# Ssellu/vslam-pose-estimation-framework

Hardware: AMD Instinct MI355X
Metric: stereo frames/sec on KITTI-00 at 1/2/4/8 MI355X; ATE vs reference (higher is better)
Workload: dtype u8

## Files before the change

vslam_pose_estimation_framework_amd/csrc/host_ctx.h:

```cpp
#pragma once

static thread_local std::string g_create_error;

#ifndef VS_SPLIT4_MAX_STREAMS
#define VS_SPLIT4_MAX_STREAMS 96
#endif
struct vslam_ctx {
  DevCfg cfg;
  DevBuf buf;
  int device = 0;
  int B = 0;
  hipStream_t stream = nullptr;
  hipStream_t stream_img = nullptr;
  bool own_stream = false;
  hipEvent_t ev_img[2] = {nullptr, nullptr}, ev_frm[2] = {nullptr, nullptr};
  bool frm_pending[2] = {false, false};
  int q0_frm = 0, q0_img = 0;
  struct ImgSet { uint16_t* box; uint8_t* score8; unsigned long long* mask; int16_t* kp_xy; uint8_t* kp_score; uint8_t* desc;
                  int32_t* n_kp; int32_t* rowcell; uint8_t* used; uint8_t* sdist; ImgInfo* iinfo; } sets[2];
  int parity = 0, last_set = 0;
  std::string err;
  std::vector<void*> allocs;
  DevCfg* d_cfg = nullptr;
  DevBuf* d_bufs = nullptr;
// ... 304 lines not shown
static void destroy_streams(vslam_ctx* c) {
  for (int q = 0; q < 2; ++q) {
    if (c->ev_img[q]) (void)hipEventDestroy(c->ev_img[q]);
    if (c->ev_frm[q]) (void)hipEventDestroy(c->ev_frm[q]);
    c->ev_img[q] = c->ev_frm[q] = nullptr;
  }
  if (c->own_stream) {
    if (c->stream_img && c->stream_img != c->stream) (void)hipStreamDestroy(c->stream_img);
    if (c->stream) (void)hipStreamDestroy(c->stream);
  }
  c->stream = c->stream_img = nullptr;
}
__global__ void k_xcc_probe(int* out) {
  unsigned v;
  asm volatile("s_getreg_b32 %0, hwreg(HW_REG_XCC_ID)" : "=s"(v));
  if (threadIdx.x == 0) *out = (int)(v & 7u);
}
static int calibrate_queues(vslam_ctx* c) {
  int* d = nullptr;
  if (hipMalloc(&d, 2 * sizeof(int)) != hipSuccess) return VSLAM_OK;
  int h[2] = {0, 0};
  hipStream_t q[2] = {c->stream, c->stream_img};
  bool ok = true;
  for (int k = 0; k < 2 && ok; ++k) { hipLaunchKernelGGL(k_xcc_probe, dim3(1), dim3(64), 0, q[k], d + k); ok = hipStreamSynchronize(q[k]) == hipSuccess; }
  if (ok && hipMemcpy(h, d, sizeof h, hipMemcpyDeviceToHost) == hipSuccess) { c->q0_frm = h[0]; c->q0_img = h[1]; }
  (void)hipFree(d);
  return VSLAM_OK;
}

static int create_internal(const vslam_config* cfg, int device, int n_streams, vslam_ctx** out) {
  if (!cfg || !out || n_streams < 1) return fail(nullptr, VSLAM_ERR_INVALID, "vslam_create: null argument or n_streams < 1");
  if (n_streams > VS_MAX_STREAMS) return fail(nullptr, VSLAM_ERR_INVALID, "vslam_create: more than 4096 streams in one context");
  if (cfg->rows < 1 || cfg->cols < 1 || cfg->cols > 32767 || cfg->rows > 32767) return fail(nullptr, VSLAM_ERR_INVALID, "vslam_create: invalid image dimensions");
  if (cfg->det_rows < 1 || cfg->det_cols < 1 || cfg->det_rows * cfg->det_cols > VSLAM_MAX_REGIONS) return fail(nullptr, VSLAM_ERR_INVALID, "vslam_create: invalid detector grid");
  if (!(-cfg->baseline_h[0] / cfg->K[0] > 0)) return fail(nullptr, VSLAM_ERR_INVALID, "vslam_create: invalid baseline (m), verify intrinsic camera parameters");
  if (cfg->maximum_epipolar_search_offset_pixels < 0 || cfg->maximum_epipolar_search_offset_pixels > VSLAM_MAX_EPI) return fail(nullptr, VSLAM_ERR_INVALID, "vslam_create: epipolar offset out of range");
  if (cfg->descriptor_type != VSLAM_DESCRIPTOR_BRIEF && cfg->descriptor_type != VSLAM_DESCRIPTOR_ORB) return fail(nullptr, VSLAM_ERR_INVALID, "vslam_create: unknown descriptor_type");
  if (cfg->max_keypoints < 64 || cfg->max_keypoints > 65535 || cfg->max_points < 64 || cfg->max_history_frames < 2 || cfg->bin_size_pixels < 1) return fail(nullptr, VSLAM_ERR_INVALID, "vslam_create: invalid capacities");
  int ndev = 0;
  if (hipGetDeviceCount(&ndev) != hipSuccess || ndev < 1) return fail(nullptr, VSLAM_ERR_NO_DEVICE, "vslam_create: no HIP device available (the HIP path has no CPU fallback)");
  if (device < 0 || device >= ndev) return fail(nullptr, VSLAM_ERR_NO_DEVICE, "vslam_create: device ordinal out of range");
  if (hipSetDevice(device) != hipSuccess) return fail(nullptr, VSLAM_ERR_NO_DEVICE, "vslam_create: hipSetDevice failed");
  hipFuncAttributes fa;
  if (hipFuncGetAttributes(&fa, reinterpret_cast<const void*>(k_frame)) != hipSuccess)
    return fail(nullptr, VSLAM_ERR_NO_DEVICE, "vslam_create: no gfx950 kernel image for this device");
  vslam_ctx* c = new vslam_ctx;
  c->device = device;
  c->B = n_streams;
  derive_cfg(*cfg, n_streams, &c->cfg);
  {
    bool ok = hipStreamCreateWithPriority(&c->stream, hipStreamNonBlocking, 0) == hipSuccess &&
              hipStreamCreateWithPriority(&c->stream_img, hipStreamNonBlocking, 0) == hipSuccess;
    if (ok && getenv("VSLAM_IMG_STREAMS") && atoi(getenv("VSLAM_IMG_STREAMS")) == 0) { (void)hipStreamDestroy(c->stream_img); c->stream_img = c->stream; }
    for (int k = 0; k < 2 && ok; ++k)
      ok = hipEventCreateWithFlags(&c->ev_img[k], hipEventDisableTiming) == hipSuccess &&
           hipEventCreateWithFlags(&c->ev_frm[k], hipEventDisableTiming) == hipSuccess;
    c->own_stream = true;
    if (!ok) { destroy_streams(c); delete c; return fail(nullptr, VSLAM_ERR_HIP, "hipStreamCreate failed"); }
    c->split = n_streams <= VS_SPLIT4_MAX_STREAMS ? 4 : 0;
    if (const char* e = getenv("VSLAM_SPLIT")) { const int v = atoi(e); if (v == 0 || v == 4) c->split = v; }
  }
  const DevCfg& d = c->cfg;
  DevBuf& b = c->buf;
  std::memset(&b, 0, sizeof b);
  std::memset(b.active, 0xff, sizeof b.active);
  const size_t B = n_streams, S2 = B * 2, rows = cfg->rows, N = d.NMAX, P = d.MAXP, Hc = d.HCAP;
// ... 242 lines not shown
```

vslam_pose_estimation_framework_amd/csrc/host_frame.h:

```cpp
#pragma once

static int report_blocks(int what) {
  return what == VS_REPORT_KEYPOINTS ? 32 : what == VS_REPORT_POINTS ? 16 : what == VS_REPORT_KEYPOINTS_XY ? 8 : 4;
}
static int report_launch(vslam_ctx* c, hipStream_t q, const DevBuf& bs, int s, int what, int in_progress) {
  const int seq = ++c->report_seq;
  hipLaunchKernelGGL(k_report, dim3(report_blocks(what)), dim3(256), 0, q, c->cfg, bs, s, what, in_progress, seq, c->rl, c->report_dev, c->report_done);
  return seq;
}
static int launch_image_pipeline(vslam_ctx* c) {
  const DevCfg& d = c->cfg;
  const int set = c->parity;
  const int n = c->B;
  hipStream_t st = c->img_override ? c->img_override : c->stream_img;
  if (!c->img_override && c->img_on_frm_queue) {
    HIP_TRY(c, hipStreamSynchronize(c->stream));
    c->img_on_frm_queue = false;
  }
  if (c->img_override) c->img_on_frm_queue = true;
  const bool coarse = c->img_override != nullptr;
  if (c->frm_pending[set] && st != c->stream) HIP_TRY(c, hipStreamWaitEvent(st, c->ev_frm[set], 0));
  HIP_TRY(c, prestage_enqueue(st, c->pre, c->rect.maps, c->eq, n, 2, c->buf.active));
  const bool masked = c->dmask.pending || c->dmask.stat[0] || c->dmask.stat[1];
  if (masked) { if (const int rc = mask_prepare(c, st)) return rc; } else c->dmask.last = 0;
// ... 142 lines not shown
  p.smooth_mode = c->sm.mode; p.smooth_ksize = c->sm.ksize;
  const ImgPlanes raw_slab = p.remap ? ImgPlanes{{r.raw[set][0], r.raw[set][1]}, r.raw_stride, r.raw_stream_stride} : p.smooth_mode ? unsmoothed_planes(c, set) : up;
  if (p.format != VSLAM_PIXEL_GRAY8) { p.color = cur; p.gray = p.factor > 1 ? ImgPlanes{{d.full[set][0], d.full[set][1]}, d.stride, d.stream_stride} : raw_slab; cur = p.gray; }
  if (p.factor > 1) { p.full = cur; p.reduced = raw_slab; cur = p.reduced; }
  if (p.remap) { p.raw = cur; p.mapped = rectified_planes(c, set); cur = p.mapped; }
  if (p.smooth_mode) { p.unsmoothed = cur; p.smoothed = c->eq.on ? ImgPlanes{{c->sm.out[0], c->sm.out[1]}, c->up_stride, c->up_stream_stride} : up; cur = p.smoothed; }
  if (c->eq.on) { c->eq.src = cur; c->eq.dst = cur.p[0] == up.p[0] ? cur : up; cur = c->eq.dst; }
  buf_set_planes(c->buf, cur);
}
static int set_inputs(vslam_ctx* c, const uint8_t* L, const uint8_t* R, int32_t row_stride, size_t image_stride, bool on_device) {
  const bool colour = c->col.format != VSLAM_PIXEL_GRAY8, full = c->ds.factor > 1, raw = c->rect.on;
  int rows, cols;
  incoming_size(c, &rows, &cols);
  const int wb = colour ? gray_channels(c->col.format) * cols : cols;
  if (!L || !R) return fail(c, VSLAM_ERR_INVALID, "called with empty frame");
  if (row_stride < wb)
    return fail(c, VSLAM_ERR_INVALID, colour ? "row stride smaller than channels * image width" : full ? "row stride smaller than the full image width" : raw ? "row stride smaller than the raw image width" : "row stride smaller than image width");
  ImgPlanes in = {{L, R}, row_stride, image_stride};
  if (!on_device) {
    if (colour && c->mapcol.rgb && c->frm_pending[c->parity]) {
      hipStream_t up[2] = {c->img_override ? c->img_override : c->stream_img, c->stream_img};
      for (int k = 0; k < 2; ++k)
        if (up[k] != c->stream && (k == 0 || up[k] != up[0])) HIP_TRY(c, hipStreamWaitEvent(up[k], c->ev_frm[c->parity], 0));
    }
    const int p = c->parity;
    const int rc = colour ? upload_to(c, L, R, row_stride, image_stride, rows, wb, c->col.slab[p], c->col.stride, c->col.stream_stride, &in)
                   : full ? upload_to(c, L, R, row_stride, image_stride, rows, cols, c->ds.full[p], c->ds.stride, c->ds.stream_stride, &in)
                   : raw  ? upload_to(c, L, R, row_stride, image_stride, rows, cols, c->rect.raw[p], c->rect.raw_stride, c->rect.raw_stream_stride, &in)
                   : c->sm.mode ? upload_to(c, L, R, row_stride, image_stride, rows, cols, c->sm.in[p], c->up_stride, c->up_stream_stride, &in)
                          : upload_to(c, L, R, row_stride, image_stride, rows, cols, c->upload[p], c->up_stride, c->up_stream_stride, &in);
    if (rc != VSLAM_OK) return rc;
  }
  route_frame(c, in);
  return VSLAM_OK;
}

static int process_frame(vslam_ctx* c, const uint8_t* L, const uint8_t* R, int32_t row_stride, size_t image_stride, bool on_device) {
  if (!c) return VSLAM_ERR_INVALID;
  if (c->sticky != VSLAM_OK) return c->sticky;
  if (!on_device) HIP_TRY(c, hipSetDevice(c->device));
  int rc = set_inputs(c, L, R, row_stride, image_stride, on_device);
  if (rc != VSLAM_OK) return rc;
  rc = flush_pending(c);
  if (rc != VSLAM_OK) return rc;
  rc = launch_image_pipeline(c);
  if (rc != VSLAM_OK) return rc;
  return launch_frame(c);
}
VS_API int vslam_process_device(vslam_ctx* c, const uint8_t* L, const uint8_t* R, int32_t row_stride, size_t image_stride) {
  return process_frame(c, L, R, row_stride, image_stride, true);
}
VS_API int vslam_process_host(vslam_ctx* c, const uint8_t* L, const uint8_t* R, int32_t row_stride, size_t image_stride) {
  return process_frame(c, L, R, row_stride, image_stride, false);
}

VS_API int vslam_host_alloc(void** out, size_t bytes) {
  if (!out || !bytes) return VSLAM_ERR_INVALID;
  void* p = nullptr;
  if (hipHostMalloc(&p, bytes, hipHostMallocDefault) != hipSuccess) { (void)hipGetLastError(); return fail(nullptr, VSLAM_ERR_HIP, "vslam_host_alloc: hipHostMalloc failed"); }
  *out = p;
  return VSLAM_OK;
}
VS_API void vslam_host_free(void* p) { if (p) (void)hipHostFree(p); }
```

vslam_pose_estimation_framework_amd/csrc/host_rgbd.h:

```cpp
#pragma once
#include "rgbd_tracker.h"
#include "rgbd_device.h"
struct vslam_rgbd {
  bool on_host = false, host_pending = false;
  int host_rc = 0;
  vs_rgbd::Tracker t;
  vs_rgbd::DeviceTracker d;
  std::string& err() { return on_host ? t.err : d.err; }
};
static thread_local std::string g_rgbd_error;
VS_API const char* vslam_rgbd_last_error(const vslam_rgbd* r) { return r ? (r->on_host ? r->t.err.c_str() : r->d.err.c_str()) : g_rgbd_error.c_str(); }
static int rgbd_create(const vslam_config* cfg, const vslam_depth_params* p, int device, int n_streams, vslam_rgbd** out) {
  if (!cfg || !p || !out) { g_rgbd_error = "vslam_rgbd_create: null argument"; return VSLAM_ERR_INVALID; }
  vslam_rgbd* r = new vslam_rgbd;
  if (const char* e = std::getenv("VSLAM_RGBD_HOST")) r->on_host = std::atoi(e) != 0;
  if (p->detector_type == VSLAM_DETECTOR_ORB) { if (!vs_rgbd::DeviceTracker::orb_grid_supported(*cfg)) r->on_host = true; }
  else if (p->detector_type != VSLAM_DETECTOR_FAST) { g_rgbd_error = "vslam_rgbd_create: unknown detector_type"; delete r; return VSLAM_ERR_INVALID; }
  if (r->on_host && n_streams != 1) { g_rgbd_error = "vslam_rgbd_create_batch: the host-driven loop (VSLAM_RGBD_HOST=1, detector_type ORB on a grid above 2 x 2) tracks one sequence per object"; delete r; return VSLAM_ERR_INVALID; }
  const int rc = r->on_host ? r->t.create(*cfg, *p, device) : r->d.create(*cfg, *p, device, n_streams);
  if (rc != VSLAM_OK) { g_rgbd_error = r->err(); delete r; return rc; }
  *out = r;
  return VSLAM_OK;
}
VS_API int vslam_rgbd_create(const vslam_config* cfg, const vslam_depth_params* p, int device, vslam_rgbd** out) { return rgbd_create(cfg, p, device, 1, out); }
VS_API int vslam_rgbd_create_batch(const vslam_config* cfg, const vslam_depth_params* p, int device, int32_t n_streams, vslam_rgbd** out) {
  return rgbd_create(cfg, p, device, n_streams, out);
}
VS_API void vslam_rgbd_destroy(vslam_rgbd* r) { delete r; }
VS_API int vslam_rgbd_reset(vslam_rgbd* r) {
  if (!r) return VSLAM_ERR_INVALID;
  if (r->on_host) { r->t.reset(); return VSLAM_OK; }
  return r->d.reset();
}
static int rgbd_frame_args_ok(vslam_rgbd* r, const uint8_t* left, int32_t lstride, const uint16_t* depth, int32_t dstride) {
  if (!left || !depth) { r->err() = "called with empty frame"; return VSLAM_ERR_INVALID; }
  const int cols = r->on_host ? r->t.cfg.cols : r->d.in_cols();
  const int wb = r->on_host ? cols : r->d.in_bytes();
  if (lstride < wb || dstride < cols) { r->err() = "row stride smaller than image width"; return VSLAM_ERR_INVALID; }
  return VSLAM_OK;
}
VS_API int vslam_rgbd_process_host(vslam_rgbd* r, const uint8_t* left, int32_t lstride, const uint16_t* depth, int32_t dstride) {
  if (!r) return VSLAM_ERR_INVALID;
  if (int rc = rgbd_frame_args_ok(r, left, lstride, depth, dstride)) return rc;
  return r->on_host ? r->t.process(left, lstride, depth, dstride) : r->d.process(left, lstride, depth, dstride);
}
VS_API int vslam_rgbd_submit_host(vslam_rgbd* r, const uint8_t* left, int32_t lstride, const uint16_t* depth, int32_t dstride) {
  if (!r) return VSLAM_ERR_INVALID;
  if (int rc = rgbd_frame_args_ok(r, left, lstride, depth, dstride)) return rc;
  if (r->on_host) { r->host_rc = r->t.process(left, lstride, depth, dstride); r->host_pending = true; return r->host_rc; }
  return r->d.submit(left, lstride, depth, dstride);
}
VS_API int vslam_rgbd_wait(vslam_rgbd* r) {
  if (!r) return VSLAM_ERR_INVALID;
  if (r->on_host) {
    if (!r->host_pending) { r->t.err = "RGB-D tracker: no frame in flight"; return VSLAM_ERR_STATE; }
    r->host_pending = false;
    return r->host_rc;
  }
  return r->d.wait();
}
VS_API int vslam_rgbd_submit_batch_host(vslam_rgbd* r, const uint8_t* left, int32_t lstride, size_t left_stream_stride, const uint16_t* depth, int32_t dstride,
                                        size_t depth_stream_stride) {
  if (!r) return VSLAM_ERR_INVALID;
  if (r->on_host) { r->t.err = "batch entry points need the device-resident loop"; return VSLAM_ERR_STATE; }
  if (int rc = rgbd_frame_args_ok(r, left, lstride, depth, dstride)) return rc;
  return r->d.submit(left, lstride, depth, dstride, left_stream_stride, depth_stream_stride);
}
VS_API int vslam_rgbd_process_batch_host(vslam_rgbd* r, const uint8_t* left, int32_t lstride, size_t left_stream_stride, const uint16_t* depth, int32_t dstride,
                                         size_t depth_stream_stride) {
  const int rc = vslam_rgbd_submit_batch_host(r, left, lstride, left_stream_stride, depth, dstride, depth_stream_stride);
  return rc != VSLAM_OK ? rc : vslam_rgbd_wait(r);
// ... 248 lines not shown
```

vslam_pose_estimation_framework_amd/csrc/kernels_image.h:

```cpp
#pragma once
#include <hip/hip_runtime.h>
#include "dev_types.h"
#include "../../include/vslam_brief_pattern.h"
#include "../../include/vslam_orb_pattern.h"
#include "brief_footprint.h"

__constant__ int8_t c_brief[256][4] = VSLAM_BRIEF_PATTERN_INIT;
constexpr int8_t k_brief_builtin[256][4] = VSLAM_BRIEF_PATTERN_INIT;
constexpr BriefFootprint k_brief_builtin_fp = brief_footprint(k_brief_builtin);
__constant__ BriefFootprint c_brief_fp = k_brief_builtin_fp;
__constant__ int8_t c_orb[256][4] = VSLAM_ORB_PATTERN_INIT;

__device__ __forceinline__ size_t ix_side(const DevCfg& c, int s, int d) { return (size_t)s * 2 + d; }
__device__ __forceinline__ uint16_t* box_of(const DevCfg& c, const DevBuf& b, int s, int d) {
  return b.box + ix_side(c, s, d) * (size_t)c.c.rows * c.bstride;
}
__device__ __forceinline__ uint8_t* score_of(const DevCfg& c, const DevBuf& b, int s, int d) {
  return b.score8 + ix_side(c, s, d) * (size_t)c.c.rows * c.bstride;
}
__device__ __forceinline__ unsigned long long* mask_of(const DevCfg& c, const DevBuf& b, int s, int d) {
  return b.mask + ix_side(c, s, d) * (size_t)c.c.rows * c.TX;
}
__device__ __forceinline__ int16_t* kpxy_of(const DevCfg& c, const DevBuf& b, int s, int d) {
  return b.kp_xy + ix_side(c, s, d) * (size_t)c.NMAX * 2;
}
__device__ __forceinline__ uint8_t* kpscore_of(const DevCfg& c, const DevBuf& b, int s, int d) {
  return b.kp_score + ix_side(c, s, d) * (size_t)c.NMAX;
}
__device__ __forceinline__ uint8_t* desc_of(const DevCfg& c, const DevBuf& b, int s, int d) {
  return b.desc + ix_side(c, s, d) * (size_t)c.NMAX * 32;
}
__device__ __forceinline__ int32_t* rowcell_of(const DevCfg& c, const DevBuf& b, int s, int d) {
  return b.rowcell + ix_side(c, s, d) * (size_t)c.c.rows * (c.CW + 1);
}
__device__ __forceinline__ uint8_t* used_of(const DevCfg& c, const DevBuf& b, int s, int d) {
  return b.used + ix_side(c, s, d) * (size_t)c.NMAX;
}
__device__ __forceinline__ int32_t* kill_of(const DevCfg& c, const DevBuf& b, int s, int d) {
  return b.kill + ix_side(c, s, d) * (size_t)c.NMAX;
}

__device__ __forceinline__ int block_exclusive_scan(int v, int* sh, int* total) {
  const int lane = threadIdx.x & 63, w = threadIdx.x >> 6, nw = blockDim.x >> 6;
  int inc = v;
#pragma unroll
  for (int o = 1; o < 64; o <<= 1) {
    const int t = __shfl_up(inc, o, 64);
    if (lane >= o) inc += t;
  }
  __syncthreads();
  if (lane == 63) sh[w] = inc;
  __syncthreads();
  if (threadIdx.x == 0) {
    int acc = 0;
    for (int i = 0; i < nw; ++i) { const int t = sh[i]; sh[i] = acc; acc += t; }
    sh[16] = acc;
  }
  __syncthreads();
  *total = sh[16];
  return sh[w] + inc - v;
}

__device__ __forceinline__ void xcd_tile(int* tx, int* ty, int* tz, int mono = 0, int rot = 0) {
  const int gx = gridDim.x, gy = gridDim.y;
  const int tps = mono ? gx * gy : gx * gy * 2;
  const int ns = mono ? gridDim.z : gridDim.z >> 1;
  int lin = blockIdx.x + gx * (blockIdx.y + gy * blockIdx.z);
  const int per = (ns >> 3) * tps;
  if (lin < (per << 3)) { const int x = (lin + rot) & 7, j = lin >> 3, q = j / tps; lin = (x + 8 * q) * tps + (j - q * tps); }
  *tx = lin % gx;
  const int r = lin / gx;
  *ty = r % gy;
// ... 45 lines not shown
__device__ __forceinline__ int lds_fetch_add(int* word, int v) {
  const uint32_t addr = (uint32_t)reinterpret_cast<uintptr_t>((__attribute__((address_space(3))) int*)word);
  int old;
  asm volatile("ds_add_rtn_u32 %0, %1, %2\n\ts_waitcnt lgkmcnt(0)" : "=&v"(old) : "v"(addr), "v"(v) : "memory");
  return old;
}

#define VS_FB_QCAP ((VS_TILE_H + 2) * 66)
#define VS_FB_HS_BYTES ((VS_TILE_H + 8) * VS_TILE_W * 2)
#define VS_FB_DYN_LDS ((VS_FB_QCAP * 2) > VS_FB_HS_BYTES ? (VS_FB_QCAP * 2) : VS_FB_HS_BYTES)
__global__ __launch_bounds__(256, 8) void k_fast_box(const DevCfg c, const DevBuf b) {
  extern __shared__ __align__(16) unsigned char fb_dyn[];
  __shared__ __align__(16) uint8_t tile[VS_TILE_H + 8][80];
  __shared__ __align__(4) uint8_t sc[VS_TILE_H + 2][68];
  __shared__ int32_t s_thr[VSLAM_MAX_REGIONS];
  uint16_t* queue = reinterpret_cast<uint16_t*>(fb_dyn);
  uint16_t (*hs)[VS_TILE_W] = reinterpret_cast<uint16_t (*)[VS_TILE_W]>(fb_dyn);
  __shared__ unsigned long long lmask[VS_TILE_H];
  __shared__ int qn;
  int tx, ty, tz;
  xcd_tile(&tx, &ty, &tz, c.mono, b.xcd_rot);
  const int s = b.s0 + (c.mono ? tz : (tz >> 1)), side = c.mono ? 0 : (tz & 1);
  if (!vs_active(b, s)) return;
  const int x0 = tx * VS_TILE_W, y0 = ty * VS_TILE_H;
  const int rows = c.c.rows, cols = c.c.cols;
  const uint8_t* img = b.img[side] + (size_t)s * b.img_stream_stride;
  const int stride = b.img_row_stride;
  const int tid = threadIdx.x, lane = tid & 63, w = tid >> 6;
  if (tid < c.n_regions) s_thr[tid] = min(max(b.st[s].thr[tid], 0), 255);
  if (tid == 0) qn = 0;
  if (tid < VS_TILE_H) lmask[tid] = 0ull;
  for (int i = tid; i < (VS_TILE_H + 2) * 17; i += 256) reinterpret_cast<uint32_t*>(&sc[0][0])[i] = 0u;
  const bool aligned = ((stride & 3) == 0) && ((reinterpret_cast<uintptr_t>(img) & 3) == 0);
  constexpr int NST = ((VS_TILE_H + 8) * 18 + 255) / 256;
  if (aligned && x0 >= 4 && x0 + 68 <= cols) {
    uint32_t v[NST];
#pragma unroll
    for (int u = 0; u < NST; ++u) {
      const int i = tid + 256 * u;
      const int r = i / 18, q = i - r * 18;
      const int gy = min(max(y0 - 4 + r, 0), rows - 1);
      v[u] = 0;
      if (i < (VS_TILE_H + 8) * 18) v[u] = __builtin_nontemporal_load(reinterpret_cast<const uint32_t*>(img + (size_t)gy * stride + (x0 - 4 + 4 * q)));
    }
#pragma unroll
    for (int u = 0; u < NST; ++u) {
      const int i = tid + 256 * u;
      const int r = i / 18, q = i - r * 18;
      if (i < (VS_TILE_H + 8) * 18) *reinterpret_cast<uint32_t*>(&tile[r][4 * q]) = v[u];
    }
  } else {
    for (int i = tid; i < (VS_TILE_H + 8) * 18; i += 256) {
      const int r = i / 18, q = i - r * 18;
      const int gy = min(max(y0 - 4 + r, 0), rows - 1), gx0 = x0 - 4 + 4 * q;
      uint32_t v = 0;
#pragma unroll
      for (int k = 0; k < 4; ++k) v |= (uint32_t)img[(size_t)gy * stride + min(max(gx0 + k, 0), cols - 1)] << (8 * k);
      *reinterpret_cast<uint32_t*>(&tile[r][4 * q]) = v;
    }
  }
  __syncthreads();
  int uni_thr = -2, vx0 = 0, vx1 = 0, vy0 = 0, vy1 = 0;
  bool uni_full = false;
  {
    int hits = 0;
    for (int r = 0; r < c.n_regions; ++r) {
      const DevRegion& R = c.regions[r];
      const int ax0 = max(R.x + 3, x0 - 1), ax1 = min(R.x + R.w - 3, x0 + 65), ay0 = max(R.y + 3, y0 - 1), ay1 = min(R.y + R.h - 3, y0 + VS_TILE_H + 1);
      if (ax0 < ax1 && ay0 < ay1) {
        if (hits == 0) { uni_thr = s_thr[r]; vx0 = ax0 - (x0 - 1); vx1 = ax1 - (x0 - 1); vy0 = ay0 - (y0 - 1); vy1 = ay1 - (y0 - 1); }
        ++hits;
      }
    }
    if (hits != 1) uni_thr = -2;
    uni_full = uni_thr != -2 && vx0 == 0 && vx1 == 66 && vy0 == 0 && vy1 == VS_TILE_H + 2;
  }
  auto pretest = [&](int r, int cc, bool valid = true) {
    const int thr = !valid ? -1 : (uni_full ? uni_thr : region_threshold(c, s_thr, x0 - 1 + cc, y0 - 1 + r));
    bool cand = false;
    if (thr >= 0) {
      const int ly = r + 3, lx = cc + 3;
      const int v = tile[ly][lx];
      const int d0 = v - tile[ly + 3][lx], d4 = v - tile[ly][lx + 3], d8 = v - tile[ly - 3][lx], d12 = v - tile[ly][lx - 3];
      const int dk = min(max(d0, d8), max(d4, d12));
      const int br = max(min(d0, d8), min(d4, d12));
      cand = dk > thr || br < -thr;
    }
    const unsigned long long m = __ballot(cand);
    if (m) {
      int base = 0;
// ... 56 lines not shown
      constexpr int NRING = 2 * 66 + 2 * VS_TILE_H;
      for (int i0 = 0; i0 < NRING; i0 += 256) {
        if (i0 + 64 * w >= NRING) continue;
        const int i = i0 + tid;
        int r = 0, cc = 0;
        if (i < 66) { r = 0; cc = i; }
        else if (i < 132) { r = VS_TILE_H + 1; cc = i - 66; }
        else { const int k = i - 132; r = 1 + (k >> 1); cc = (k & 1) ? 65 : 0; }
        pretest(r, cc, i < NRING);
      }
    } else {
      if (tid >= 64 && tid < 64 + (VS_TILE_H + 2) * 2) { const int i = tid - 64; pretest(i >> 1, (i & 1) ? 65 : 0); }
    }
  } else {
    for (int r = w; r < VS_TILE_H + 2; r += 4) pretest(r, lane);
    if (tid < (VS_TILE_H + 2) * 2) pretest(tid >> 1, 64 + (tid & 1));
    static_assert((VS_TILE_H + 2) * 2 <= 256, "one pass over the halo columns");
  }
  __syncthreads();
  {
    const int nq = qn;
    for (int q = tid; 2 * q < nq; q += 256) {
      const int e0 = queue[2 * q], e1 = (2 * q + 1 < nq) ? queue[2 * q + 1] : e0;
      const int r0 = e0 >> 8, c0 = e0 & 255, r1 = e1 >> 8, c1 = e1 & 255;
      int sv0, sv1;
      const int t0 = uni_thr != -2 ? uni_thr : region_threshold(c, s_thr, x0 - 1 + c0, y0 - 1 + r0);
      const int t1 = uni_thr != -2 ? uni_thr : region_threshold(c, s_thr, x0 - 1 + c1, y0 - 1 + r1);
      fast_pair_scores(tile, r0 + 3, c0 + 3, r1 + 3, c1 + 3, t0, t1, &sv0, &sv1);
      sc[r0][c0] = (uint8_t)sv0;
      if (2 * q + 1 < nq) sc[r1][c1] = (uint8_t)sv1;
    }
  }
  __syncthreads();
  unsigned long long* mask = mask_of(c, b, s, side);
  uint8_t* score8 = score_of(c, b, s, side);
  uint16_t* box = box_of(c, b, s, side);
  {
    const int nq = qn;
    for (int q = tid; q < nq; q += 256) {
      const int e0 = queue[q];
      const int r = e0 >> 8, cc = e0 & 255;
      if (r < 1 || r > VS_TILE_H || cc < 1 || cc > 64) continue;
      const int v = sc[r][cc];
      if (v == 0) continue;
      const bool keep = v > sc[r - 1][cc - 1] && v > sc[r - 1][cc] && v > sc[r - 1][cc + 1] && v > sc[r][cc - 1] &&
                        v > sc[r][cc + 1] && v > sc[r + 1][cc - 1] && v > sc[r + 1][cc] && v > sc[r + 1][cc + 1];
      if (keep) {
        atomicOr(&lmask[r - 1], 1ull << (cc - 1));
        const int gy = y0 + r - 1;
        if (gy < rows) score8[(size_t)gy * c.bstride + (x0 + cc - 1)] = (uint8_t)v;
      }
    }
  }
  __syncthreads();
  const bool want_box = c.c.descriptor_type == VSLAM_DESCRIPTOR_BRIEF;
  if (want_box)
  for (int i = tid; i < (VS_TILE_H + 8) * 16; i += 256) {
    const int r = i >> 4, q = i & 15;
    const uint32_t* p = reinterpret_cast<const uint32_t*>(&tile[r][4 * q]);
    const uint32_t w0 = p[0], w1 = p[1], w2 = p[2];
    const uint32_t s0 = __builtin_amdgcn_sad_u8(w0, 0u, __builtin_amdgcn_sad_u8(w1, 0u, w2 & 255u));
    const uint32_t s1 = s0 - (w0 & 255u) + ((w2 >> 8) & 255u);
    const uint32_t s2 = s1 - ((w0 >> 8) & 255u) + ((w2 >> 16) & 255u);
    const uint32_t s3 = s2 - ((w0 >> 16) & 255u) + (w2 >> 24);
    *reinterpret_cast<uint2*>(&hs[r][4 * q]) = make_uint2(s0 | (s1 << 16), s2 | (s3 << 16));
  }
  __syncthreads();
  if (want_box) {
    constexpr int RW = VS_TILE_H / 8;
    const int half = lane >> 5, px = 2 * (lane & 31);
    const int rbase = (w * 2 + half) * RW;
    typedef unsigned short u16x2 __attribute__((ext_vector_type(2)));
    u16x2 acc = {0, 0};
#pragma unroll
    for (int k = 0; k < 9; ++k) acc += *reinterpret_cast<const u16x2*>(&hs[rbase + k][px]);
#pragma unroll
    for (int j = 0; j < RW; ++j) {
      const int r = rbase + j, gy = y0 + r;
      if (gy < rows && x0 + px < c.bstride) __builtin_nontemporal_store(__builtin_bit_cast(uint32_t, acc), reinterpret_cast<uint32_t*>(box + (size_t)gy * c.bstride + x0 + px));
      if (j < RW - 1) acc += *reinterpret_cast<const u16x2*>(&hs[r + 9][px]) - *reinterpret_cast<const u16x2*>(&hs[r][px]);
    }
  }
  __syncthreads();
  if (tid < VS_TILE_H && y0 + tid < rows) mask[(size_t)(y0 + tid) * c.TX + tx] = lmask[tid];
}

__device__ __forceinline__ unsigned long long col_mask(int lo, int hi, int wx0) {
  const int a = min(max(lo - wx0, 0), 64), e = min(max(hi - wx0, 0), 64);
  const unsigned long long from_a = a >= 64 ? 0ull : (~0ull << a), below_e = e >= 64 ? ~0ull : ~(~0ull << e);
  return from_a & below_e;
}

__device__ __forceinline__ int wave_scan_incl(int x) {
  int s = x;
  s += __builtin_amdgcn_update_dpp(0, x, 0x111, 0xf, 0xf, false);
  s += __builtin_amdgcn_update_dpp(0, x, 0x112, 0xf, 0xf, false);
  s += __builtin_amdgcn_update_dpp(0, x, 0x113, 0xf, 0xf, false);
  s += __builtin_amdgcn_update_dpp(0, s, 0x114, 0xf, 0xe, false);
  s += __builtin_amdgcn_update_dpp(0, s, 0x118, 0xf, 0xc, false);
  s += __builtin_amdgcn_update_dpp(0, s, 0x142, 0xa, 0xf, false);
  s += __builtin_amdgcn_update_dpp(0, s, 0x143, 0xc, 0xf, false);
  return s;
}
__device__ __forceinline__ int wave_sum(int x) { return __builtin_amdgcn_readlane(wave_scan_incl(x), 63); }

#ifndef VS_EMIT_WPT
#define VS_EMIT_WPT 4
#endif
#define VS_EMIT_THREADS 256
#define VS_EMIT_BAND (VS_EMIT_THREADS * VS_EMIT_WPT)
#define VS_EMIT_PF 8
#define VS_EMIT_HEAD 2
__global__ __launch_bounds__(VS_EMIT_THREADS, 8) void k_emit(const DevCfg c, const DevBuf b, int border, int run_controller) {
  __shared__ int sh_pre[VS_EMIT_THREADS / 64], sh_own[VS_EMIT_THREADS / 64];
  __shared__ int sh_cnt[VS_EMIT_THREADS / 64][VSLAM_MAX_REGIONS];
  const int side = blockIdx.y, band = (int)gridDim.z - 1 - (int)blockIdx.z, tid = threadIdx.x;
  const int s = b.s0 + xcd_local_stream(blockIdx.x, gridDim.x, (int)((b.xcd_rot + (side + gridDim.y * blockIdx.z) * gridDim.x) & 7));
// ... 192 lines not shown
#define VS_BT_H 64
#endif
#define VS_BT_RW (VS_BT_W + 2 * VSLAM_BRIEF_PATCH_HALF)
#define VS_BT_RH (VS_BT_H + 2 * VSLAM_BRIEF_PATCH_HALF)
__global__ __launch_bounds__(256) void k_brief(const DevCfg c, const DevBuf b) {
  __shared__ __align__(16) uint16_t reg[VS_BT_RH * VS_BT_RW];
  __shared__ int row_lo[VS_BT_H], row_off[VS_BT_H + 1];
  int tx, ty, tz;
  xcd_tile(&tx, &ty, &tz, c.mono, b.xcd_rot);
  const int s = b.s0 + (c.mono ? tz : (tz >> 1)), side = c.mono ? 0 : (tz & 1);
  if (!vs_active(b, s)) return;
  const int x0 = tx * VS_BT_W, y0 = ty * VS_BT_H;
  const int rows = c.c.rows;
  const int tid = threadIdx.x, lane = tid & 63, w = tid >> 6;
  const int32_t* rowcell = rowcell_of(c, b, s, side);
  if (tid < VS_BT_H) {
    const int r = y0 + tid;
    int lo = 0, n = 0;
    if (r < rows) {
      const int c0 = min((VS_BT_W / 16) * tx, c.CW), c1 = min((VS_BT_W / 16) * (tx + 1), c.CW);
      lo = rowcell[(size_t)r * (c.CW + 1) + c0];
      n = rowcell[(size_t)r * (c.CW + 1) + c1] - lo;
    }
    row_lo[tid] = lo;
    int inc = n;
#pragma unroll
    for (int o = 1; o < VS_BT_H; o <<= 1) { const int t = __shfl_up(inc, o, 64); if (tid >= o) inc += t; }
    row_off[tid + 1] = inc;
    if (tid == 0) row_off[0] = 0;
  }
  __syncthreads();
  const int K = row_off[VS_BT_H];
  if (K == 0) return;
  const uint16_t* box = box_of(c, b, s, side);
  constexpr int CPR = VS_BT_RW / 8;
  constexpr int NLD = (VS_BT_RH * CPR + 255) / 256;
  uint4 stage[NLD];
#pragma unroll
  for (int u = 0; u < NLD; ++u) {
    const int i = tid + 256 * u;
    const int r = i / CPR, q = i - r * CPR;
    const int gy = min(max(y0 - VSLAM_BRIEF_PATCH_HALF + r, 0), rows - 1);
    const int gx = x0 - VSLAM_BRIEF_PATCH_HALF + 8 * q;
    stage[u] = make_uint4(0u, 0u, 0u, 0u);
    if (i < VS_BT_RH * CPR && gx >= 0 && gx + 8 <= c.bstride) stage[u] = *reinterpret_cast<const uint4*>(box + (size_t)gy * c.bstride + gx);
  }
  const int16_t* kxy = kpxy_of(c, b, s, side);
  auto lookup = [&](int k, int* base, int* idx) {
    *base = 0; *idx = -1;
    if (k < K) {
      int r = 0;
#pragma unroll
      for (int step = VS_BT_H / 2; step > 0; step >>= 1) if (row_off[r + step] <= k) r += step;
      const int id = row_lo[r] + (k - row_off[r]);
      *idx = id;
      *base = (r + VSLAM_BRIEF_PATCH_HALF) * VS_BT_RW + (kxy[2 * id] - x0 + VSLAM_BRIEF_PATCH_HALF);
    }
  };
  int my_base, my_idx;
  lookup(w + 4 * lane, &my_base, &my_idx);
  int off_a[4], off_b[4];
#pragma unroll
  for (int j = 0; j < 4; ++j) {
    const int i = j * 64 + lane;
    off_a[j] = c_brief[i][0] * VS_BT_RW + c_brief[i][1];
    off_b[j] = c_brief[i][2] * VS_BT_RW + c_brief[i][3];
  }
#pragma unroll
  for (int u = 0; u < NLD; ++u) {
    const int i = tid + 256 * u;
    if (i < VS_BT_RH * CPR) *reinterpret_cast<uint4*>(&reg[8 * i]) = stage[u];
  }
  __syncthreads();
  uint8_t* desc = desc_of(c, b, s, side);
  for (int k0 = 0; k0 < K; k0 += 256) {
    if (k0 > 0) lookup(k0 + w + 4 * lane, &my_base, &my_idx);
    const int n_here = (min(K - k0, 256) - w + 3) >> 2;
    for (int i = 0; i < n_here; ++i) {
      const int base = __builtin_amdgcn_readlane(my_base, i), idx = __builtin_amdgcn_readlane(my_idx, i);
      unsigned long long word = 0;
#pragma unroll
      for (int j = 0; j < 4; ++j) {
        const unsigned long long m = __ballot(reg[base + off_a[j]] < reg[base + off_b[j]]);
        if (lane == j) word = m;
      }
      if (lane < 4) reinterpret_cast<unsigned long long*>(desc + (size_t)32 * idx)[lane] = __builtin_bswap64(__brevll(word));
    }
  }
}

__global__ __launch_bounds__(256) void k_brief_at(const uint16_t* box, int bstride, int rows, int cols, int n,
                                                  const int16_t* xy, uint8_t* keep, uint8_t* desc) {
  const int lane = threadIdx.x & 63;
  const int wave = blockIdx.x * (blockDim.x >> 6) + (threadIdx.x >> 6);
  const int nwaves = gridDim.x * (blockDim.x >> 6);
  for (int i = wave; i < n; i += nwaves) {
    const int x = xy[2 * i], y = xy[2 * i + 1];
    const bool in = x >= VSLAM_BRIEF_BORDER && x < cols - VSLAM_BRIEF_BORDER && y >= VSLAM_BRIEF_BORDER && y < rows - VSLAM_BRIEF_BORDER;
    if (lane == 0) keep[i] = in ? 1 : 0;
    if (in) brief_wave(box, bstride, x, y, lane, desc + (size_t)32 * i);
    else if (lane < 4) reinterpret_cast<unsigned long long*>(desc + (size_t)32 * i)[lane] = 0ull;
  }
}

struct Gauss7 { int32_t k[4]; };
__device__ __forceinline__ int reflect101(int p, int n) { return p < 0 ? -p : (p >= n ? 2 * n - 2 - p : p); }
__device__ __forceinline__ uint8_t* blur_of(const DevCfg& c, const DevBuf& b, int s, int d) { return reinterpret_cast<uint8_t*>(box_of(c, b, s, d)); }

__device__ __forceinline__ void gauss7_tile(const uint8_t* img, int stride, int rows, int cols, int x0, int y0, const Gauss7& g, uint8_t* out, int ostride,
                                            uint8_t (*src)[72], uint16_t (*hs)[VS_TILE_W]) {
  const int tid = threadIdx.x;
  const bool in_dwords = ((stride & 3) == 0) && ((reinterpret_cast<uintptr_t>(img) & 3) == 0) && x0 >= 4 && x0 + 68 <= cols;
  if (in_dwords) {
    constexpr int NST = ((VS_TILE_H + 6) * 18 + 255) / 256;
    uint32_t v[NST];
#pragma unroll
    for (int u = 0; u < NST; ++u) {
      const int i = tid + 256 * u;
// ... 301 lines not shown
```

Baseline: 198,300.

## Use 32-bit plane offsets, incremental staging plans, and scalar-uniform bases in image kernels

Adds a StagingPlan helper that walks tile staging loads with incremental 32-bit byte offsets instead of per-item division and 64-bit address math, with a fast unclamped path for interior tiles in both the FAST box kernel and the BRIEF tile kernel. Per-plane base pointers are forced into scalar registers with readfirstlane, and row clamping uses v_med3. The BRIEF descriptor word assembly replaces four lane-conditional selects with inline v_writelane. New host checks reject planes of 2^31 bytes or more so the 32-bit offsets stay valid, which limits the image sizes the library accepts.

```diff
diff --git a/vslam_pose_estimation_framework_amd/csrc/host_ctx.h b/vslam_pose_estimation_framework_amd/csrc/host_ctx.h
--- a/vslam_pose_estimation_framework_amd/csrc/host_ctx.h
+++ b/vslam_pose_estimation_framework_amd/csrc/host_ctx.h
@@ -360,6 +360,8 @@
   if (!cfg || !out || n_streams < 1) return fail(nullptr, VSLAM_ERR_INVALID, "vslam_create: null argument or n_streams < 1");
   if (n_streams > VS_MAX_STREAMS) return fail(nullptr, VSLAM_ERR_INVALID, "vslam_create: more than 4096 streams in one context");
   if (cfg->rows < 1 || cfg->cols < 1 || cfg->cols > 32767 || cfg->rows > 32767) return fail(nullptr, VSLAM_ERR_INVALID, "vslam_create: invalid image dimensions");
+  if (!plane_fits_32(cfg->rows, 2 * (int64_t)((cfg->cols + VS_TILE_W - 1) / VS_TILE_W * VS_TILE_W)))
+    return fail(nullptr, VSLAM_ERR_INVALID, "vslam_create: box plane too large: rows * padded cols * 2 must stay below 2^31 bytes");
   if (cfg->det_rows < 1 || cfg->det_cols < 1 || cfg->det_rows * cfg->det_cols > VSLAM_MAX_REGIONS) return fail(nullptr, VSLAM_ERR_INVALID, "vslam_create: invalid detector grid");
   if (!(-cfg->baseline_h[0] / cfg->K[0] > 0)) return fail(nullptr, VSLAM_ERR_INVALID, "vslam_create: invalid baseline (m), verify intrinsic camera parameters");
   if (cfg->maximum_epipolar_search_offset_pixels < 0 || cfg->maximum_epipolar_search_offset_pixels > VSLAM_MAX_EPI) return fail(nullptr, VSLAM_ERR_INVALID, "vslam_create: epipolar offset out of range");
diff --git a/vslam_pose_estimation_framework_amd/csrc/host_frame.h b/vslam_pose_estimation_framework_amd/csrc/host_frame.h
--- a/vslam_pose_estimation_framework_amd/csrc/host_frame.h
+++ b/vslam_pose_estimation_framework_amd/csrc/host_frame.h
@@ -198,6 +198,8 @@
     if (rc != VSLAM_OK) return rc;
   }
   route_frame(c, in);
+  if (!plane_fits_32(c->cfg.c.rows, c->buf.img_row_stride))
+    return fail(c, VSLAM_ERR_INVALID, "image plane too large: rows * row stride must stay below 2^31 bytes");
   return VSLAM_OK;
 }
 
diff --git a/vslam_pose_estimation_framework_amd/csrc/host_rgbd.h b/vslam_pose_estimation_framework_amd/csrc/host_rgbd.h
--- a/vslam_pose_estimation_framework_amd/csrc/host_rgbd.h
+++ b/vslam_pose_estimation_framework_amd/csrc/host_rgbd.h
@@ -37,6 +37,7 @@
   const int cols = r->on_host ? r->t.cfg.cols : r->d.in_cols();
   const int wb = r->on_host ? cols : r->d.in_bytes();
   if (lstride < wb || dstride < cols) { r->err() = "row stride smaller than image width"; return VSLAM_ERR_INVALID; }
+  if (!r->on_host && !plane_fits_32(r->d.in_rows(), lstride)) { r->err() = "image plane too large: rows * row stride must stay below 2^31 bytes"; return VSLAM_ERR_INVALID; }
   return VSLAM_OK;
 }
 VS_API int vslam_rgbd_process_host(vslam_rgbd* r, const uint8_t* left, int32_t lstride, const uint16_t* depth, int32_t dstride) {
diff --git a/vslam_pose_estimation_framework_amd/csrc/kernels_image.h b/vslam_pose_estimation_framework_amd/csrc/kernels_image.h
--- a/vslam_pose_estimation_framework_amd/csrc/kernels_image.h
+++ b/vslam_pose_estimation_framework_amd/csrc/kernels_image.h
@@ -1,9 +1,11 @@
 #pragma once
 #include <hip/hip_runtime.h>
+#include <type_traits>
 #include "dev_types.h"
 #include "../../include/vslam_brief_pattern.h"
 #include "../../include/vslam_orb_pattern.h"
 #include "brief_footprint.h"
+#include "staging_plan.h"
 
 __constant__ int8_t c_brief[256][4] = VSLAM_BRIEF_PATTERN_INIT;
 constexpr int8_t k_brief_builtin[256][4] = VSLAM_BRIEF_PATTERN_INIT;
@@ -38,6 +40,13 @@
 }
 __device__ __forceinline__ int32_t* kill_of(const DevCfg& c, const DevBuf& b, int s, int d) {
   return b.kill + ix_side(c, s, d) * (size_t)c.NMAX;
+}
+
+template <class T>
+__device__ __forceinline__ T* uniform_base(T* all, T* p) {
+  const size_t o = (size_t)(p - all);
+  const uint32_t lo = __builtin_amdgcn_readfirstlane((uint32_t)o), hi = __builtin_amdgcn_readfirstlane((uint32_t)(o >> 32));
+  return all + (((size_t)hi << 32) | lo);
 }
 
 __device__ __forceinline__ int block_exclusive_scan(int v, int* sh, int* total) {
@@ -149,30 +158,41 @@
   if (tid < VS_TILE_H) lmask[tid] = 0ull;
   for (int i = tid; i < (VS_TILE_H + 2) * 17; i += 256) reinterpret_cast<uint32_t*>(&sc[0][0])[i] = 0u;
   const bool aligned = ((stride & 3) == 0) && ((reinterpret_cast<uintptr_t>(img) & 3) == 0);
-  constexpr int NST = ((VS_TILE_H + 8) * 18 + 255) / 256;
+  using Plan = StagingPlan<VS_TILE_H + 8, 18>;
+  constexpr int NST = Plan::LOADS;
   if (aligned && x0 >= 4 && x0 + 68 <= cols) {
     uint32_t v[NST];
+    auto load_all = [&](auto unclamped) {
+      Plan pl = Plan::first(tid);
+      pl.row += y0 - 4;
+      uint32_t off = plane_offset(clamp_row(pl.row, rows), stride, x0 - 4 + 4 * pl.chunk);
+      const uint32_t inc = Plan::step_bytes((uint32_t)stride, 4u), more = Plan::carry_bytes((uint32_t)stride, 4u);
+#pragma unroll
+      for (int u = 0; u < NST; ++u) {
+        v[u] = 0;
+        if (Plan::has(tid, u)) v[u] = __builtin_nontemporal_load(reinterpret_cast<const uint32_t*>(img + off));
+        const bool carry = pl.carries();
+        pl.step();
+        if (decltype(unclamped)::value) off += inc + (carry ? more : 0u);
+        else off = plane_offset(clamp_row(pl.row, rows), stride, x0 - 4 + 4 * pl.chunk);
+      }
+    };
+    if (y0 >= 4 && y0 + VS_TILE_H + 4 <= rows) load_all(std::true_type()); else load_all(std::false_type());
+    Plan pl = Plan::first(tid);
+    uint32_t lo = (uint32_t)(pl.row * 80 + 4 * pl.chunk);
 #pragma unroll
     for (int u = 0; u < NST; ++u) {
-      const int i = tid + 256 * u;
+      if (Plan::has(tid, u)) *reinterpret_cast<uint32_t*>(&tile[0][0] + lo) = v[u];
+      lo += Plan::step_bytes(80u, 4u) + (pl.carries() ? Plan::carry_bytes(80u, 4u) : 0u);
+      pl.step();
+    }
+  } else {
+    for (int i = tid; i < Plan::ITEMS; i += 256) {
       const int r = i / 18, q = i - r * 18;
-      const int gy = min(max(y0 - 4 + r, 0), rows - 1);
-      v[u] = 0;
-      if (i < (VS_TILE_H + 8) * 18) v[u] = __builtin_nontemporal_load(reinterpret_cast<const uint32_t*>(img + (size_t)gy * stride + (x0 - 4 + 4 * q)));
-    }
-#pragma unroll
-    for (int u = 0; u < NST; ++u) {
-      const int i = tid + 256 * u;
-      const int r = i / 18, q = i - r * 18;
-      if (i < (VS_TILE_H + 8) * 18) *reinterpret_cast<uint32_t*>(&tile[r][4 * q]) = v[u];
-    }
-  } else {
-    for (int i = tid; i < (VS_TILE_H + 8) * 18; i += 256) {
-      const int r = i / 18, q = i - r * 18;
-      const int gy = min(max(y0 - 4 + r, 0), rows - 1), gx0 = x0 - 4 + 4 * q;
+      const int gy = clamp_row(y0 - 4 + r, rows), gx0 = x0 - 4 + 4 * q;
       uint32_t v = 0;
 #pragma unroll
-      for (int k = 0; k < 4; ++k) v |= (uint32_t)img[(size_t)gy * stride + min(max(gx0 + k, 0), cols - 1)] << (8 * k);
+      for (int k = 0; k < 4; ++k) v |= (uint32_t)img[plane_offset(gy, stride, min(max(gx0 + k, 0), cols - 1))] << (8 * k);
       *reinterpret_cast<uint32_t*>(&tile[r][4 * q]) = v;
     }
   }
@@ -295,9 +315,9 @@
     }
   }
   __syncthreads();
-  unsigned long long* mask = mask_of(c, b, s, side);
-  uint8_t* score8 = score_of(c, b, s, side);
-  uint16_t* box = box_of(c, b, s, side);
+  unsigned long long* mask = uniform_base(b.mask, mask_of(c, b, s, side));
+  uint8_t* score8 = uniform_base(b.score8, score_of(c, b, s, side));
+  uint16_t* box = uniform_base(b.box, box_of(c, b, s, side));
   {
     const int nq = qn;
     for (int q = tid; q < nq; q += 256) {
@@ -311,7 +331,7 @@
       if (keep) {
         atomicOr(&lmask[r - 1], 1ull << (cc - 1));
         const int gy = y0 + r - 1;
-        if (gy < rows) score8[(size_t)gy * c.bstride + (x0 + cc - 1)] = (uint8_t)v;
+        if (gy < rows) score8[plane_offset(gy, c.bstride, x0 + cc - 1)] = (uint8_t)v;
       }
     }
   }
@@ -337,15 +357,20 @@
     u16x2 acc = {0, 0};
 #pragma unroll
     for (int k = 0; k < 9; ++k) acc += *reinterpret_cast<const u16x2*>(&hs[rbase + k][px]);
+    const uint32_t row_bytes = (uint32_t)c.bstride * 2u;
+    uint32_t off = plane_offset(y0 + rbase, (int)row_bytes, 2 * (x0 + px));
+    const int nrow = x0 + px < c.bstride ? rows - (y0 + rbase) : 0;
+    uint8_t* boxb = reinterpret_cast<uint8_t*>(box);
 #pragma unroll
     for (int j = 0; j < RW; ++j) {
-      const int r = rbase + j, gy = y0 + r;
-      if (gy < rows && x0 + px < c.bstride) __builtin_nontemporal_store(__builtin_bit_cast(uint32_t, acc), reinterpret_cast<uint32_t*>(box + (size_t)gy * c.bstride + x0 + px));
+      const int r = rbase + j;
+      if (j < nrow) __builtin_nontemporal_store(__builtin_bit_cast(uint32_t, acc), reinterpret_cast<uint32_t*>(boxb + off));
+      off += row_bytes;
       if (j < RW - 1) acc += *reinterpret_cast<const u16x2*>(&hs[r + 9][px]) - *reinterpret_cast<const u16x2*>(&hs[r][px]);
     }
   }
   __syncthreads();
-  if (tid < VS_TILE_H && y0 + tid < rows) mask[(size_t)(y0 + tid) * c.TX + tx] = lmask[tid];
+  if (tid < VS_TILE_H && y0 + tid < rows) *reinterpret_cast<unsigned long long*>(reinterpret_cast<uint8_t*>(mask) + plane_offset(y0 + tid, c.TX * 8, tx * 8)) = lmask[tid];
 }
 
 __device__ __forceinline__ unsigned long long col_mask(int lo, int hi, int wx0) {
@@ -604,19 +629,33 @@
   __syncthreads();
   const int K = row_off[VS_BT_H];
   if (K == 0) return;
-  const uint16_t* box = box_of(c, b, s, side);
-  constexpr int CPR = VS_BT_RW / 8;
-  constexpr int NLD = (VS_BT_RH * CPR + 255) / 256;
-  uint4 stage[NLD];
-#pragma unroll
-  for (int u = 0; u < NLD; ++u) {
-    const int i = tid + 256 * u;
-    const int r = i / CPR, q = i - r * CPR;
-    const int gy = min(max(y0 - VSLAM_BRIEF_PATCH_HALF + r, 0), rows - 1);
-    const int gx = x0 - VSLAM_BRIEF_PATCH_HALF + 8 * q;
-    stage[u] = make_uint4(0u, 0u, 0u, 0u);
-    if (i < VS_BT_RH * CPR && gx >= 0 && gx + 8 <= c.bstride) stage[u] = *reinterpret_cast<const uint4*>(box + (size_t)gy * c.bstride + gx);
-  }
+  using Plan = StagingPlan<VS_BT_RH, VS_BT_RW / 8>;
+  constexpr int NLD = Plan::LOADS;
+  const uint8_t* boxb = reinterpret_cast<const uint8_t*>(uniform_base(b.box, box_of(c, b, s, side)));
+  const uint32_t row_bytes = (uint32_t)c.bstride * 2u;
+  const int xb0 = 2 * (x0 - VSLAM_BRIEF_PATCH_HALF);
+  const int qlo = x0 < VSLAM_BRIEF_PATCH_HALF ? (VSLAM_BRIEF_PATCH_HALF - x0 + 7) / 8 : 0;
+  const int qhi = min(VS_BT_RW / 8, (c.bstride - x0 + VSLAM_BRIEF_PATCH_HALF) / 8);
+  const bool plain = y0 >= VSLAM_BRIEF_PATCH_HALF && y0 + VS_BT_H + VSLAM_BRIEF_PATCH_HALF <= rows && qlo == 0 && qhi == VS_BT_RW / 8;
+  typedef uint32_t u32x4 __attribute__((ext_vector_type(4)));
+  u32x4 stage[NLD];
+  bool in_row[NLD];
+  auto load_all = [&](auto is_plain) {
+    Plan pl = Plan::first(tid);
+    pl.row += y0 - VSLAM_BRIEF_PATCH_HALF;
+    uint32_t off = plane_offset(clamp_row(pl.row, rows), (int)row_bytes, xb0 + 16 * pl.chunk);
+    const uint32_t inc = Plan::step_bytes(row_bytes, 16u), more = Plan::carry_bytes(row_bytes, 16u);
+#pragma unroll
+    for (int u = 0; u < NLD; ++u) {
+      in_row[u] = decltype(is_plain)::value || (unsigned)(pl.chunk - qlo) < (unsigned)(qhi - qlo);
+      if (Plan::has(tid, u) && in_row[u]) stage[u] = *reinterpret_cast<const u32x4*>(boxb + off);
+      const bool carry = pl.carries();
+      pl.step();
+      if (decltype(is_plain)::value) off += inc + (carry ? more : 0u);
+      else off = plane_offset(clamp_row(pl.row, rows), (int)row_bytes, xb0 + 16 * pl.chunk);
+    }
+  };
+  if (plain) load_all(std::true_type()); else load_all(std::false_type());
   const int16_t* kxy = kpxy_of(c, b, s, side);
   auto lookup = [&](int k, int* base, int* idx) {
     *base = 0; *idx = -1;
@@ -638,24 +677,33 @@
     off_a[j] = c_brief[i][0] * VS_BT_RW + c_brief[i][1];
     off_b[j] = c_brief[i][2] * VS_BT_RW + c_brief[i][3];
   }
+  const u32x4 zero4 = {0u, 0u, 0u, 0u};
 #pragma unroll
   for (int u = 0; u < NLD; ++u) {
-    const int i = tid + 256 * u;
-    if (i < VS_BT_RH * CPR) *reinterpret_cast<uint4*>(&reg[8 * i]) = stage[u];
+    if (!Plan::has(tid, u)) continue;
+    u32x4* dst = reinterpret_cast<u32x4*>(&reg[8 * (tid + 256 * u)]);
+    if (in_row[u]) *dst = stage[u]; else *dst = zero4;
   }
   __syncthreads();
   uint8_t* desc = desc_of(c, b, s, side);
+  uint32_t word_lo = 0, word_hi = 0;
   for (int k0 = 0; k0 < K; k0 += 256) {
     if (k0 > 0) lookup(k0 + w + 4 * lane, &my_base, &my_idx);
     const int n_here = (min(K - k0, 256) - w + 3) >> 2;
     for (int i = 0; i < n_here; ++i) {
       const int base = __builtin_amdgcn_readlane(my_base, i), idx = __builtin_amdgcn_readlane(my_idx, i);
-      unsigned long long word = 0;
-#pragma unroll
-      for (int j = 0; j < 4; ++j) {
-        const unsigned long long m = __ballot(reg[base + off_a[j]] < reg[base + off_b[j]]);
-        if (lane == j) word = m;
-      }
+      unsigned long long m[4];
+#pragma unroll
+      for (int j = 0; j < 4; ++j) m[j] = __ballot(reg[base + off_a[j]] < reg[base + off_b[j]]);
+      asm("s_nop 4\n\t"
+          "v_writelane_b32 %0, %2, 0\n\tv_writelane_b32 %1, %3, 0\n\t"
+          "v_writelane_b32 %0, %4, 1\n\tv_writelane_b32 %1, %5, 1\n\t"
+          "v_writelane_b32 %0, %6, 2\n\tv_writelane_b32 %1, %7, 2\n\t"
+          "v_writelane_b32 %0, %8, 3\n\tv_writelane_b32 %1, %9, 3"
+          : "+v"(word_lo), "+v"(word_hi)
+          : "s"((uint32_t)m[0]), "s"((uint32_t)(m[0] >> 32)), "s"((uint32_t)m[1]), "s"((uint32_t)(m[1] >> 32)),
+            "s"((uint32_t)m[2]), "s"((uint32_t)(m[2] >> 32)), "s"((uint32_t)m[3]), "s"((uint32_t)(m[3] >> 32)));
+      const unsigned long long word = ((unsigned long long)word_hi << 32) | word_lo;
       if (lane < 4) reinterpret_cast<unsigned long long*>(desc + (size_t)32 * idx)[lane] = __builtin_bswap64(__brevll(word));
     }
   }
diff --git a/vslam_pose_estimation_framework_amd/csrc/staging_plan.h b/vslam_pose_estimation_framework_amd/csrc/staging_plan.h
--- /dev/null
+++ b/vslam_pose_estimation_framework_amd/csrc/staging_plan.h
@@ -0,0 +1,40 @@
+#pragma once
+#include <stdint.h>
+#include "exp_fixed.h"
+
+#define VS_STAGE_THREADS 256
+#define VS_PLANE_LIMIT 0x80000000ull
+
+VS_XD inline bool plane_fits_32(int64_t rows, int64_t row_bytes) {
+  return rows >= 0 && row_bytes >= 0 && (uint64_t)rows * (uint64_t)row_bytes < VS_PLANE_LIMIT;
+}
+VS_XD inline uint32_t plane_offset(int gy, int stride, int xb) { return (uint32_t)gy * (uint32_t)stride + (uint32_t)xb; }
+VS_XD inline int clamp_row(int y, int rows) {
+#if defined(__HIP_DEVICE_COMPILE__)
+  int r;
+  asm("v_med3_i32 %0, %1, 0, %2" : "=v"(r) : "v"(y), "v"(rows - 1));
+  return r;
+#else
+  return y < 0 ? 0 : (y > rows - 1 ? rows - 1 : y);
+#endif
+}
+
+template <int RH, int CPR>
+struct StagingPlan {
+  static constexpr int NT = VS_STAGE_THREADS;
+  static constexpr int ITEMS = RH * CPR;
+  static constexpr int LOADS = (ITEMS + NT - 1) / NT;
+  static constexpr int DROW = NT / CPR, DCHUNK = NT % CPR;
+  static_assert(CPR >= 1 && CPR <= NT, "a step of 256 items carries at most once");
+  int row, chunk;
+  VS_XD static constexpr StagingPlan first(int tid) { return StagingPlan{tid / CPR, tid % CPR}; }
+  VS_XD constexpr void step() {
+    row += DROW; chunk += DCHUNK;
+    if (chunk >= CPR) { chunk -= CPR; ++row; }
+  }
+  VS_XD constexpr bool carries() const { return chunk + DCHUNK >= CPR; }
+  VS_XD static constexpr uint32_t step_bytes(uint32_t row_bytes, uint32_t chunk_bytes) { return (uint32_t)DROW * row_bytes + (uint32_t)DCHUNK * chunk_bytes; }
+  VS_XD static constexpr uint32_t carry_bytes(uint32_t row_bytes, uint32_t chunk_bytes) { return row_bytes - (uint32_t)CPR * chunk_bytes; }
+  VS_XD static constexpr bool has(int tid, int u) { return u < LOADS - 1 || tid + NT * u < ITEMS; }
+  VS_XD constexpr bool inside() const { return row < RH; }
+};
```

Result: no change. 199,400 (median of 6 runs) (+0.6%).
